# PalamaraLab/FastSMC

Hardware: NVIDIA B200
Metric: hmm_pair_sites_per_s (higher is better)
Workload: dtype f32

## Files before the change

fastsmc_b200/csrc/capi.cu:

```cuda
#include <algorithm>
#include <atomic>
#include <cub/device/device_radix_sort.cuh>
#include <chrono>
#include <cstdarg>
#include <cstdint>
#include <cstdio>
#include <cstdlib>
#include <cstring>
#include <map>
#include <tuple>
#include <numeric>
#include <string>
#include <thread>
#include <vector>

#include "decode_kernels.cuh"
#include "decode_fast.cuh"
#include "decode_sparse.cuh"
#include "seed_kernels.cuh"
#include "seed_order.h"
#include "host/SeedMapOrder.hpp"
#include "segment_sort.h"
#include "split_select.h"

// ... 71 lines not shown
    if (e == cudaSuccess) {
      n = want;
    }
    return e;
  }
};

}

struct fsmc_plan;

struct SeedKey {
  int32_t gap;
  float minLengthCm;
  uint64_t genPosSum, globalIdSum, flipSum;
  float skip;
  uint32_t window[4];
  int32_t lastJob, aboveDiag;
  uint32_t flags;
  int32_t maxSeeds, readAhead;
};

struct fsmc_ctx {
  int device = 0;
  cudaStream_t ownStream = nullptr;
  cudaStream_t stream = nullptr;
  cudaDeviceProp prop{};
  bool hasModel = false, hasHaps = false;
  uint64_t modelTag = 0;
  fsmc::DeviceModel model{};
  fsmc::DeviceModel kernelModel{};
  DevBuf<float> kernelSiteRows;
  DevBuf<float> laneAux;
  DevBuf<float> siteRows, prior, expTimes, colRatios;
  DevBuf<uint64_t> haps;
  long long numHaps = 0;
  DevBuf<float> scratch, accScratch;
  DevBuf<float> stageE1, stageE0, stageE2, stageD, stageB, stageU, stageR;
  DevBuf<int> stageRowIdx;
  DevBuf<float> sumScratch;
  DevBuf<float> ckptBeta;
  std::vector<float> hostPrior, hostExpTimes, hostColRatios;
  long long sites = 0;
  DevBuf<uint64_t> seedKeysT;
  DevBuf<uint32_t> seedOwner, seedSlotCount, seedSlotGroup, seedSlotOf, seedRankOf, seedMembers, seedGroupSize,
      seedGroupMemberBase, seedGlobalId;
  DevBuf<unsigned long long> seedGroupPairBase, seedCounters, seedWordCounters, seedChunkBase;
  DevBuf<float> seedGenPos;
  DevBuf<fsmc_match> seedOut;
  DevBuf<uint32_t> seedRank;
  DevBuf<unsigned char> seedLowComplexity;
  DevBuf<uint32_t> seedRep0, seedCur;
  DevBuf<unsigned char> seedDepth;
  DevBuf<uint64_t> seedRegKeyT, seedRegKeys;
  fsmc::CandidateOrderer orderer;
  const fsmc_match* orderedOut = nullptr;
  bool seedCacheValid = false;
  SeedKey seedCacheKey{};
  fsmc_seed_stats seedCacheStats{};
  cudaEvent_t ev[4] = {nullptr, nullptr, nullptr, nullptr};
  PinnedBuf<fsmc_segment> segStage;
  std::vector<uint32_t> pairOffset, pairFirst;
  fsmc::SegmentSorter segmentSorter;
  fsmc_plan* sparePlan = nullptr;
  std::map<std::tuple<const void*, int, size_t>, int> occupancy;
};
// ... 105 lines not shown
    }
    return {};
  }
  const bool acc = (flags & FSMC_SEG_AGE) && (flags & FSMC_CALL_SEGMENTS);
  const bool narrow = !(flags & (FSMC_SITE_MEAN | FSMC_SITE_MAP | FSMC_WIDE_KERNEL)) && (!acc || m.ageThreshold <= m.stateThreshold) &&
                      m.stateThreshold + 1 <= 4 * fsmc::kNarrowMaxQuads;
  const int rqWanted = narrow ? (m.stateThreshold + 1 + 3) / 4 : 0;
  const int pref = (flags & FSMC_ONE_WARP_KERNEL) ? 0 : splitPreference();
  const bool trySplit = pref == 1 || (pref == -1 && S == 159);
  if (trySplit && (S == 69 || S == 159) && m.stateThreshold <= 32) {
    fsmc::SplitChoice sc{};
    static const bool laneOff = [] { const char* e = std::getenv("FSMC_LANE"); return e && *e == '0'; }();
    if (S == 159 && m.laneAux && !laneOff) {
      sc = fsmc::laneKernel159(rqWanted);
    }
    if (!sc.fn) {
      sc = S == 69 ? fsmc::splitKernel69(rqWanted, acc) : fsmc::splitKernel159(rqWanted, acc);
    }
    if (!sc.fn && narrow) {
      sc = S == 69 ? fsmc::splitKernel69(0, acc) : fsmc::splitKernel159(0, acc);
    }
    if (sc.fn) {
      FastChoice fc{sc.fn, sc.Spad, sc.warps * 32, sc.acc, sc.recordQuads > 0, sc.recordQuads};
      fc.splitWarps = sc.warps;
      fc.splitSmem = sc.smemBytes;
      return fc;
    }
  }
  const bool sparse = preferSparse && S == 69 && acc && m.ageThreshold > m.stateThreshold &&
                      !(flags & (FSMC_SITE_MEAN | FSMC_SITE_MAP | FSMC_WIDE_KERNEL)) && m.stateThreshold + 1 <= 4 * fsmc::kNarrowMaxQuads;
  if (sparse) {
    const int rq = (m.stateThreshold + 1 + 3) / 4;
    FastKernelFn fn = rq == 1   ? fsmc::decodeNarrowKernel<69, 1, 4, kFastDepth, 128, 2, 1>
                      : rq == 2 ? fsmc::decodeNarrowKernel<69, 2, 4, kFastDepth, 128, 2, 1>
                      : rq == 3 ? fsmc::decodeNarrowKernel<69, 3, 2, kFastDepth, 128, 2, 1>
                                : fsmc::decodeNarrowKernel<69, 4, 2, kFastDepth, 128, 2, 1>;
    if (const char* e = std::getenv("FSMC_SPARSE_VARIANT")) {
      const int v = std::atoi(e);
      if (rq == 1 && v == 65) fn = fsmc::decodeNarrowKernel<69, 1, 4, kFastDepth, 128, 2, 65>;
    }
    FastChoice fc{fn, 72, 128, false, true, rq};
    fc.sparse = true;
    return fc;
  }
  if (S == 69 && narrow) {
    const int rq = (m.stateThreshold + 1 + 3) / 4;
    FastKernelFn fn = rq == 1   ? fsmc::decodeNarrowKernel<69, 1, 4, kFastDepth, 128, 2>
                      : rq == 2 ? fsmc::decodeNarrowKernel<69, 2, 4, kFastDepth, 128, 2>
                      : rq == 3 ? fsmc::decodeNarrowKernel<69, 3, 2, kFastDepth, 128, 2>
                                : fsmc::decodeNarrowKernel<69, 4, 2, kFastDepth, 128, 2>;
    if (const char* e = std::getenv("FSMC_SPARSE_VARIANT")) {
      if (rq == 1 && std::atoi(e) == 65) fn = fsmc::decodeNarrowKernel<69, 1, 4, kFastDepth, 128, 2, 64>;
    }
    return FastChoice{fn, 72, 128, false, true, rq};
  }
  if (S == 69) {
    return acc ? FastChoice{fsmc::decodeFastKernel<69, kFastDepth, kFastRescale, true, 128, 2>, 72, 128, true}
               : FastChoice{fsmc::decodeFastKernel<69, kFastDepth, kFastRescale, false, 128, 2>, 72, 128, false};
  }
  return {};
}
bool sparsePreferred(const double meanScanSites)
{
  if (const char* e = std::getenv("FSMC_SPARSE")) {
    return std::atoi(e) != 0;
  }
  return meanScanSites >= 2000.0;
}

size_t fastSmemBytes(const FastChoice& fc, const int S)
{
  if (fc.splitWarps > 0) {
    return fc.splitSmem;
  }
  const size_t warps = fc.threads / 32;
  if (fc.narrow) {
    const size_t group = fc.recordQuads <= 2 ? 4 : 2;
    const size_t slot = group * static_cast<size_t>(fsmc::kRowArrays) * fc.Spad * 4 + (group + 1) * static_cast<size_t>(fc.recordQuads) * 32 * 16;
    return warps * kFastDepth * slot + warps * kFastDepth * sizeof(uint64_t);
  }
  return warps * (kFastDepth * (static_cast<size_t>(fc.Spad) * 32 * 4 + static_cast<size_t>(fsmc::kRowArrays) * fc.Spad * 4) +
                  0 * static_cast<size_t>(S)) +
         warps * 2 * kFastDepth * sizeof(uint64_t);
}

size_t sumPosteriorCount(const DeviceModel& m, const unsigned flags)
{
  return static_cast<size_t>((flags & FSMC_SUM_BY_GENOTYPE) ? 3 : 1) * static_cast<size_t>(m.S) * static_cast<size_t>(m.L);
}

size_t smemPerWarp(const DeviceModel& m, const int mode, const unsigned flags)
{
  const bool age = (flags & FSMC_SEG_AGE) && (flags & FSMC_CALL_SEGMENTS);
  const size_t rows = (age ? m.ageThreshold : 0) + (mode >= 1 ? m.S : 0) + (mode == 2 ? m.S : 0);
  return rows * 32 * sizeof(float);
}

}

extern "C" {

const char* fsmc_last_error(void)
{
  return gLastError.c_str();
}

int fsmc_version(void)
{
  return 100;
}

// ... 147 lines not shown
  const int threads = 256;
  const int blocks = std::max(1, ctx->prop.multiProcessorCount * 8);
  fsmc::buildSiteRowsKernel<<<blocks, threads, 0, st>>>(S, Spad, L, e1.p, e0.p, e2.p, D.p, B.p, U.p, R.p, rowIdx.p,
                                                         ctx->siteRows.p);
  FSMC_CUDA(cudaGetLastError());
  FSMC_CUDA(cudaStreamSynchronize(st));

  DeviceModel& m = ctx->model;
  m.S = S;
  m.Spad = Spad;
  m.L = L;
  m.siteRows = ctx->siteRows.p;
  m.prior = ctx->prior.p;
  m.expTimes = ctx->expTimes.p;
  m.colRatios = ctx->colRatios.p;
  setThresholds(m);
  m.haps = ctx->haps.p;
  m.wordsPerHap = ctx->hasHaps ? (ctx->sites + 63) / 64 : 0;
  ctx->kernelModel = m;
  const int Sk = S <= 69 ? 69 : (S <= 159 ? 159 : 0);
  if (Sk != 0 && Sk != S) {
    const int SpadK = (Sk + 3) / 4 * 4;
    FSMC_CUDA(ctx->kernelSiteRows.ensure(static_cast<size_t>(L) * fsmc::kRowArrays * SpadK));
    fsmc::buildSiteRowsKernel<<<blocks, threads, 0, st>>>(S, SpadK, L, e1.p, e0.p, e2.p, D.p, B.p, U.p, R.p, rowIdx.p,
                                                           ctx->kernelSiteRows.p);
    FSMC_CUDA(cudaGetLastError());
    FSMC_CUDA(cudaStreamSynchronize(st));
    ctx->kernelModel.S = Sk;
    ctx->kernelModel.Spad = SpadK;
    ctx->kernelModel.siteRows = ctx->kernelSiteRows.p;
  }
  ctx->model.laneAux = nullptr;
  ctx->kernelModel.laneAux = nullptr;
  if (ctx->kernelModel.S == 159) {
    FSMC_CUDA(ctx->laneAux.ensure(static_cast<size_t>(L) * fsmc::laneAuxFloats159()));
    fsmc::buildLaneAux159(L, ctx->kernelModel.siteRows, ctx->laneAux.p, blocks, st);
    FSMC_CUDA(cudaGetLastError());
    FSMC_CUDA(cudaStreamSynchronize(st));
    ctx->kernelModel.laneAux = ctx->laneAux.p;
  }
  ctx->hasModel = true;
  ctx->modelTag = mdl->modelTag;
  return FSMC_OK;
}

int fsmc_set_haplotypes(fsmc_ctx* ctx, const uint64_t* bits, const int64_t numHaps, const int64_t sites)
{
  if (!ctx || !bits || numHaps < 1 || sites < 1) {
    return fail(FSMC_E_INVALID, "fsmc_set_haplotypes: bad argument");
  }
  FSMC_CUDA(cudaSetDevice(ctx->device));
  const long long words = (sites + 63) / 64;
  const size_t n = static_cast<size_t>(numHaps) * words;
  FSMC_CUDA(ctx->haps.ensure(n));
  FSMC_CUDA(cudaMemcpyAsync(ctx->haps.p, bits, n * sizeof(uint64_t), cudaMemcpyHostToDevice, ctx->stream));
  FSMC_CUDA(cudaStreamSynchronize(ctx->stream));
  ctx->model.haps = ctx->haps.p;
  ctx->model.wordsPerHap = words;
  ctx->kernelModel.haps = ctx->haps.p;
  ctx->kernelModel.wordsPerHap = words;
  ctx->numHaps = numHaps;
  ctx->sites = sites;
  ctx->hasHaps = true;
  ctx->seedCacheValid = false;
  return FSMC_OK;
}
// ... 990 lines not shown
```

fastsmc_b200/csrc/decode_fast.cuh:

```cuda
#pragma once

#include "decode_kernels.cuh"

namespace fsmc
{

constexpr int kMaxParamStates = 160;

struct FastModel {
  DeviceModel base;
  float colRatios[kMaxParamStates];
  float expTimes[kMaxParamStates];
  float prior[kMaxParamStates];
};

__device__ __forceinline__ uint32_t smemPtr(const void* p)
{
  return static_cast<uint32_t>(__cvta_generic_to_shared(p));
}
__device__ __forceinline__ void mbarInit(uint64_t* bar, const uint32_t count)
{
  asm volatile("mbarrier.init.shared::cta.b64 [%0], %1;" ::"r"(smemPtr(bar)), "r"(count) : "memory");
}
__device__ __forceinline__ void mbarExpectTx(uint64_t* bar, const uint32_t bytes)
// ... 248 lines not shown
          const float2 t = __fmul2_rn(pk(f4(u4, 2 * jp), f4(u4, 2 * jp + 1)), xx);
          const float au0 = au;
          const float au1 = fmaf(colRatios[k], au0, t.x);
          au = fmaf(colRatios[k1], au1, t.y);
          const float2 tt = __ffma2_rn(pk(f4(d4, 2 * jp), f4(d4, 2 * jp + 1)), xx, pk(au0, au1));
          const float2 w = __fmul2_rn(pk(f4(e4, 2 * jp), f4(e4, 2 * jp + 1)),
                                      __ffma2_rn(pk(f4(b4, 2 * jp), f4(b4, 2 * jp + 1)), pk(y[k], y[k1]), tt));
          y[k] = w.x;
          y[k1] = w.y;
        } else if (k < S) {
          y[k] = f4(e4, 2 * jp) * fmaf(f4(d4, 2 * jp), x[k], au);
        }
      }
    }
    {
      const int ql = QM - 1 - i;
      const float4 e4 = E[ql], b4 = Br[ql];
#pragma unroll
      for (int jp = 1; jp >= 0; --jp) {
        const int k = 4 * ql + 2 * jp, k1 = k + 1;
        const float s1 = run;
        const float s0 = s1 + x[k1];
        run = s0 + x[k];
        const float2 w = __fmul2_rn(pk(f4(e4, 2 * jp), f4(e4, 2 * jp + 1)),
                                    __ffma2_rn(pk(f4(b4, 2 * jp), f4(b4, 2 * jp + 1)), pk(s0, s1), pk(y[k], y[k1])));
        y[k] = w.x;
        y[k1] = w.y;
      }
    }
  }
  return run;
}

static __device__ __noinline__ int emitSparseItems(SparseItem* items, float* itemAlpha, unsigned long long* itemCount,
                                            const long long capacity, const bool pred, const uint32_t pair, const int block,
                                            const int first, const int last, int chain, const float4* alphaStart,
                                            const int lane, const int SQ)
{
  const unsigned mask = __ballot_sync(kFull, pred);
  if (!mask) {
    return chain;
  }
  unsigned long long base = 0;
  if (lane == 0) {
    base = atomicAdd(itemCount, static_cast<unsigned long long>(__popc(mask)));
  }
  base = __shfl_sync(kFull, base, 0);
  if (pred) {
    const long long slot = static_cast<long long>(base) + __popc(mask & ((1u << lane) - 1u));
    if (slot < capacity) {
      items[slot] = SparseItem{pair, block, first, last, chain};
      float4* dst = reinterpret_cast<float4*>(itemAlpha + static_cast<size_t>(slot) * SQ * 4);
      for (int q = 0; q < SQ; ++q) {
        dst[q] = alphaStart[q * 32 + lane];
      }
    }
    chain = static_cast<int>(slot);
  }
  return chain;
}

constexpr int kNarrowMaxQuads = 4;
constexpr int kNarrowGroup = 4;

template <int S_T, int RQ, int G> struct NarrowSlot {
  static constexpr int SQ = (S_T + 3) / 4, Spad = SQ * 4;
  static constexpr uint32_t kCoefBytes = kRowArrays * Spad * 4;
  static constexpr uint32_t kRecBytes = RQ * 32 * 16;
  static constexpr uint32_t kBytes = G * kCoefBytes + (G + 1) * kRecBytes;
};

template <int S_T, int RQ, int G, int DEPTH, int THREADS, int MIN_BLOCKS, int SPARSE_V = 0>
__global__ void __launch_bounds__(THREADS, MIN_BLOCKS) decodeNarrowKernel(const FastModel fm, const DecodeArgs args)
{
  constexpr bool SPARSE = (SPARSE_V & 1) != 0;
  constexpr bool kSkipFwd = (SPARSE_V & 2) != 0, kSkipBwd = (SPARSE_V & 4) != 0;
  constexpr int kGroupUnroll = (SPARSE_V & 64) ? G / 2 : 1;
  constexpr bool kSkipAlpha = (SPARSE_V & 8) != 0, kSkipBoundaryItems = (SPARSE_V & 16) != 0, kSkipRunItems = (SPARSE_V & 32) != 0;
  constexpr int S = S_T;
  constexpr int SQ = (S + 3) / 4;
  constexpr int Spad = SQ * 4;
  constexpr int NR = 4 * RQ - 1;
  using Slot = NarrowSlot<S_T, RQ, G>;
  constexpr uint32_t kRecBytes = Slot::kRecBytes;
  constexpr uint32_t kCoefBytes = Slot::kCoefBytes;
  constexpr size_t kRecFloats = static_cast<size_t>(RQ) * 32 * 4;
  constexpr size_t kRowFloats = static_cast<size_t>(kRowArrays) * Spad;
  constexpr int kWarps = THREADS / 32;
  constexpr size_t kWarpBytes = static_cast<size_t>(DEPTH) * Slot::kBytes;
  static_assert(S >= 4 * kNarrowMaxQuads && RQ >= 1 && RQ <= kNarrowMaxQuads, "record quads index the state vector");
  static_assert(G % 2 == 0, "the two state vectors swap roles every step");

  extern __shared__ __align__(128) unsigned char smemRaw[];
  const DeviceModel m = fm.base;
  const int lane = threadIdx.x & 31;
  const int warp = threadIdx.x >> 5;
  unsigned char* mine = smemRaw + static_cast<size_t>(warp) * kWarpBytes;
  uint64_t* bars = reinterpret_cast<uint64_t*>(smemRaw + static_cast<size_t>(kWarps) * kWarpBytes) + warp * DEPTH;
  auto coefArea = [&](const int slot) { return reinterpret_cast<float*>(mine + static_cast<size_t>(slot) * Slot::kBytes); };
  auto recArea = [&](const int slot) {
    return reinterpret_cast<float4*>(mine + static_cast<size_t>(slot) * Slot::kBytes + static_cast<size_t>(G) * kCoefBytes);
  };
  if (lane == 0) {
    for (int i = 0; i < DEPTH; ++i) {
      mbarInit(&bars[i], 1);
    }
    asm volatile("fence.mbarrier_init.release.cluster;" ::: "memory");
  }
  __syncwarp();
  uint32_t parity = 0;

  const unsigned flags = args.flags;
  const bool wantSeg = flags & FSMC_CALL_SEGMENTS;
  const bool wantAge = !SPARSE && (flags & FSMC_SEG_AGE) && wantSeg;
  const int sT = m.stateThreshold;
  const long long warpGlobal = static_cast<long long>(blockIdx.x) * kWarps + warp;
  float* slab = args.scratch + warpGlobal * args.scratchPerWarp;
  constexpr size_t kVecFloats = static_cast<size_t>(SQ) * 32 * 4;
  const int ckShift = SPARSE ? args.ckptShift : 0;
  const int ckMask = (1 << ckShift) - 1;
// ... 34 lines not shown
    };

    float a[S], c[S];
    float acc[NR];
#pragma unroll
    for (int k = 0; k < NR; ++k) {
      acc[k] = 0.f;
    }

    auto stageRecord = [&](const float (&v)[S], float4* out, const float divisor) {
#pragma unroll
      for (int q = 0; q < RQ; ++q) {
        float w[4];
#pragma unroll
        for (int i = 0; i < 4; ++i) {
          const int k = 4 * q + i;
          w[i] = k == NR ? divisor : (k < sT ? v[k] : 0.f);
        }
        out[q * 32 + lane] = make_float4(w[0], w[1], w[2], w[3]);
      }
    };

    {
      const int steps = len - 1;
      const int first = SPARSE ? min(steps, (len % G) ? (len % G) : G) : G;
      const int nGroups = steps <= 0 ? 0 : 1 + (max(steps - first, 0) + G - 1) / G;
      auto groupBegin = [&](const int g) { return g == 0 ? 0 : first + (g - 1) * G; };
      auto prefetch = [&](const int g) {
        if (lane == 0) {
          const int j0 = groupBegin(g), j1 = min(steps, j0 + (g == 0 ? first : G));
          const int slot = g % DEPTH;
          const uint32_t bytes = static_cast<uint32_t>(j1 - j0) * kCoefBytes;
          mbarExpectTx(&bars[slot], bytes);
          bulkLoad(coefArea(slot), rowBase + static_cast<size_t>(len - j1) * kRowFloats, bytes, &bars[slot]);
        }
      };
      for (int g = 0; g < DEPTH && g < nGroups; ++g) {
        prefetch(g);
      }
#pragma unroll
      for (int k = 0; k < S; ++k) {
        a[k] = 1.f;
      }
      if constexpr (SPARSE) {
        storeCheckpoint(a, len - 1);
      }
      if (nGroups == 0) {
        stageRecord(a, recArea(0), 1.0f);
        fenceProxyAsync();
        __syncwarp();
        if (lane == 0) {
          bulkStore(slab, recArea(0), kRecBytes);
          bulkCommit();
        }
      }
      for (int g = 0; g < nGroups; ++g) {
        const int slot = g % DEPTH;
        const int j0 = groupBegin(g);
        const int n = min(g == 0 ? first : G, steps - j0);
        const float* coef = coefArea(slot);
        float4* stage = recArea(slot);
        if constexpr (SPARSE && !kSkipBwd) {
          if (g > 0 && ((len - 1 - j0) & ckMask) == ckMask) {
            storeCheckpoint(a, len - 1 - j0);
          }
        }
        if (lane == 0) {
          bulkWaitRead<DEPTH - 1>();
        }
        mbarWait(&bars[slot], (parity >> slot) & 1u);
        parity ^= 1u << slot;
        __syncwarp();
        if (g == 0) {
          stageRecord(a, stage + static_cast<size_t>(n) * RQ * 32, 1.0f);
        }
        auto step = [&](const int i, float (&x)[S], float (&y)[S], const bool rescale) {
          const int p = len - 2 - (j0 + i);
          const int cls = bits.cls(from + p + 1);
          backwardStep<S>(x, y, coef + static_cast<size_t>(n - 1 - i) * kRowFloats, cls);
          float divisor = 1.0f;
          if (rescale) {
            divisor = sumStates<S>(y);
            scaleStates<S>(y, 1.0f / divisor);
          }
          stageRecord(y, stage + static_cast<size_t>(n - 1 - i) * RQ * 32, divisor);
        };
#pragma unroll(kGroupUnroll)
        for (int i = 0; i < G; i += 2) {
          if (i < n) {
            step(i, a, c, false);
          }
          if (i + 1 < n) {
            step(i + 1, c, a, i + 1 == G - 1);
          }
        }
        fenceProxyAsync();
        __syncwarp();
        if (lane == 0) {
          const int j1 = j0 + n;
          bulkStore(slab + static_cast<size_t>(len - 1 - j1) * kRecFloats, stage,
                    static_cast<uint32_t>(n + (g == 0 ? 1 : 0)) * kRecBytes);
          bulkCommit();
        }
        if (g + DEPTH < nGroups) {
          prefetch(g + DEPTH);
        }
        if (SPARSE && g == 0 && (n & 1)) {
#pragma unroll
          for (int k = 0; k < S; ++k) {
            a[k] = c[k];
          }
        }
      }
      const int rest = SPARSE ? max(steps - first, 0) : steps;
      if (rest & 1) {
      } else {
#pragma unroll
        for (int k = 0; k < S; ++k) {
          c[k] = a[k];
        }
      }
      if (lane == 0) {
        bulkWaitAll<0>();
      }
      __syncwarp();
    }

    {
      const int nGroups = (len + G - 1) / G;
      auto prefetch = [&](const int g) {
        if (lane == 0) {
          const int p0 = g * G;
          const uint32_t n = static_cast<uint32_t>(min(G, len - p0));
          const int slot = g % DEPTH;
          mbarExpectTx(&bars[slot], n * (kCoefBytes + kRecBytes));
          bulkLoad(coefArea(slot), rowBase + static_cast<size_t>(p0) * kRowFloats, n * kCoefBytes, &bars[slot]);
          bulkLoad(recArea(slot), slab + static_cast<size_t>(p0) * kRecFloats, n * kRecBytes, &bars[slot]);
        }
      };
      for (int g = 0; g < DEPTH && g < nGroups; ++g) {
        prefetch(g);
      }
      CallerState cs;
      float Z = 1.f, bPrev = 1.f;
      bool runOpen = false;
      int pieceStart = 0, chain = -1;
      auto emitItems = [&](const bool pred, const int block, const int first, const int last) {
        chain = emitSparseItems(args.items, args.itemAlpha, args.itemCount, args.itemCapacity, pred, pair, block, first, last, chain,
                                alphaStart, lane, SQ);
      };

      auto consume = [&](const int p, const float (&v)[S], float4* rec) {
        const int site = from + p;
        float q[4 * RQ];
#pragma unroll
        for (int qq = 0; qq < RQ; ++qq) {
          const float4 r4 = rec[qq * 32 + lane];
#pragma unroll
          for (int i = 0; i < 4; ++i) {
            q[4 * qq + i] = f4(r4, i);
          }
        }
        bPrev = q[NR];
        float ibdRaw = 0.f;
#pragma unroll
        for (int k = 0; k < NR; ++k) {
          q[k] *= v[k];
          ibdRaw += q[k];
        }
        const float r = 1.0f / Z;
        const float ibd = ibdRaw * r;
        if ((flags & FSMC_SITE_IBD) && laneActive) {
          args.siteIbd[static_cast<size_t>(pair) * args.siteStride + p] = ibd;
        }
        const bool inScan = wantSeg && site >= scanFrom && site < scanTo;
        if (inScan) {
          int now = ibd >= m.thr[0] ? 0 : (ibd >= m.thr[1] ? 1 : (ibd >= m.thr[2] ? 2 : (ibd >= m.thr[3] ? 3 : -1)));
          if (!laneActive) {
            now = -1;
          }
          const bool changed = now != cs.level;
          const bool ending = changed && cs.level >= 0;
          const bool closing = now >= 0 && site == scanTo - 1;
          const float rr = now >= 0 ? r : 0.f;
          const float keep = changed ? 0.f : 1.f;
          if constexpr (SPARSE && !kSkipFwd) {
            if (__any_sync(kFull, ending || closing)) {
              if constexpr (!kSkipRunItems) {
                emitItems(ending && runOpen && pieceStart <= site - 1, (p - 1) >> ckShift, pieceStart, site - 1);
              }
              if (ending) {
                emitSegment<false>(m, args, pair, cs.start, site - 1, cs.prob, cs.level, nullptr, false, chain);
                chain = -1;
                runOpen = false;
              }
              if (now >= 0 && changed) {
                runOpen = true;
                pieceStart = site;
              }
              if constexpr (!kSkipRunItems) {
                emitItems(closing, p >> ckShift, pieceStart, site);
              }
              if (closing) {
                emitSegment<false>(m, args, pair, changed ? site : cs.start, site, changed ? ibd : cs.prob + ibd, now, nullptr,
                                   false, chain);
                chain = -1;
                runOpen = false;
              }
            } else if (now >= 0 && changed) {
              runOpen = true;
              pieceStart = site;
            }
          } else if (__any_sync(kFull, ending || closing)) {
            float* park = reinterpret_cast<float*>(rec) + lane;
            __syncwarp();
            if (wantAge) {
#pragma unroll
              for (int k = 0; k < NR; ++k) {
                park[k * 32] = acc[k];
              }
              __syncwarp();
            }
            if (ending) {
              emitSegment<false>(m, args, pair, cs.start, site - 1, cs.prob, cs.level, park, wantAge);
            }
            __syncwarp();
            if (wantAge) {
#pragma unroll
              for (int k = 0; k < NR; ++k) {
                acc[k] = fmaf(q[k], rr, keep * acc[k]);
                park[k * 32] = acc[k];
              }
              __syncwarp();
            }
            if (closing) {
              emitSegment<false>(m, args, pair, changed ? site : cs.start, site, changed ? ibd : cs.prob + ibd, now, park, wantAge);
            }
            __syncwarp();
          } else if (wantAge) {
#pragma unroll
            for (int k = 0; k < NR; ++k) {
              acc[k] = fmaf(q[k], rr, keep * acc[k]);
            }
          }
          cs.prob = (now >= 0 && !closing) ? (changed ? ibd : cs.prob + ibd) : 0.f;
          cs.start = (now >= 0 && changed) ? site : cs.start;
          cs.level = now;
        }
      };

      for (int g = 0; g < nGroups; ++g) {
        const int slot = g % DEPTH;
        const int p0 = g * G;
        const int n = min(G, len - p0);
        const float* coef = coefArea(slot);
        float4* recs = recArea(slot);
        mbarWait(&bars[slot], (parity >> slot) & 1u);
        parity ^= 1u << slot;
        if constexpr (SPARSE && !kSkipFwd) {
          if (g > 0 && (p0 & ckMask) == 0) {
            if constexpr (!kSkipBoundaryItems) {
              if (__any_sync(kFull, runOpen)) {
                emitItems(runOpen, (p0 - 1) >> ckShift, pieceStart, from + p0 - 1);
              }
            }
            pieceStart = from + p0;
            if constexpr (!kSkipAlpha) {
              storeVector(c, alphaStart);
            }
          }
        }
        auto step = [&](const int i, float (&x)[S], float (&y)[S], const bool rescale) {
          const int p = p0 + i;
          const int cls = bits.cls(from + p);
          const float total = forwardStep<S>(fm.colRatios, x, y, coef + static_cast<size_t>(i) * kRowFloats, cls);
          float sc = 1.0f;
          if (rescale) {
            sc = 1.0f / total;
            scaleStates<S>(y, sc);
          }
          Z *= bPrev * sc;
          consume(p, y, recs + static_cast<size_t>(i) * RQ * 32);
        };
#pragma unroll(kGroupUnroll)
        for (int i = 0; i < G; i += 2) {
          if (i == 0 && g == 0) {
            const int cls = bits.cls(from);
            const float4* E = reinterpret_cast<const float4*>(coef + cls * Spad);
            float z0 = 0.f, z1 = 0.f, z2 = 0.f, z3 = 0.f;
#pragma unroll
            for (int q = 0; q < SQ; ++q) {
              const float4 e4 = E[q];
#pragma unroll
              for (int j = 0; j < 4; ++j) {
                const int k = 4 * q + j;
                if (k < S) {
                  a[k] = fm.prior[k] * f4(e4, j);
                }
              }
              z0 = fmaf(a[4 * q], c[4 * q], z0);
              if (4 * q + 1 < S) z1 = fmaf(a[4 * q + 1], c[4 * q + 1], z1);
              if (4 * q + 2 < S) z2 = fmaf(a[4 * q + 2], c[4 * q + 2], z2);
              if (4 * q + 3 < S) z3 = fmaf(a[4 * q + 3], c[4 * q + 3], z3);
            }
            Z = (z0 + z1) + (z2 + z3);
            consume(0, a, recs);
          } else if (i < n) {
            step(i, c, a, false);
          }
          if (i + 1 < n) {
            step(i + 1, a, c, i + 1 == G - 1);
          }
        }
        __syncwarp();
        if (g + DEPTH < nGroups) {
          prefetch(g + DEPTH);
        }
      }
    }
    __syncwarp();
  }
}

template <int S_T, int DEPTH, int RESCALE, bool ACC, int THREADS, int MIN_BLOCKS, bool SUM = false>
__global__ void __launch_bounds__(THREADS, MIN_BLOCKS) decodeFastKernel(const FastModel fm, const DecodeArgs args)
{
  constexpr int S = S_T;
  constexpr int SQ = (S + 3) / 4;
  constexpr int Spad = SQ * 4;
  constexpr uint32_t kBetaBytes = SQ * 32 * 16;
  constexpr uint32_t kCoefBytes = kRowArrays * Spad * 4;
  constexpr size_t kBetaFloats = static_cast<size_t>(SQ) * 32 * 4;
  constexpr int kWarps = THREADS / 32;
  constexpr size_t kWarpBytes = static_cast<size_t>(DEPTH) * (kBetaBytes + kCoefBytes);

  extern __shared__ __align__(128) unsigned char smemRaw[];
  const DeviceModel m = fm.base;
  const int lane = threadIdx.x & 31;
  const int warp = threadIdx.x >> 5;
  unsigned char* mine = smemRaw + static_cast<size_t>(warp) * kWarpBytes;
  uint64_t* bars = reinterpret_cast<uint64_t*>(smemRaw + static_cast<size_t>(kWarps) * kWarpBytes) +
                   warp * 2 * DEPTH;
  auto betaSlot = [&](const int i) { return reinterpret_cast<float4*>(mine + static_cast<size_t>(i) * kBetaBytes); };
  auto coefSlot = [&](const int i) {
    return reinterpret_cast<const float*>(mine + static_cast<size_t>(DEPTH) * kBetaBytes + static_cast<size_t>(i) * kCoefBytes);
  };
  if (lane == 0) {
    for (int i = 0; i < 2 * DEPTH; ++i) {
      mbarInit(&bars[i], 1);
// ... 365 lines not shown
```

fastsmc_b200/csrc/decode_kernels.cuh:

```cuda
#pragma once

#include <cstdint>
#include <cuda_runtime.h>

#include "../../include/fastsmc_b200.h"

namespace fsmc
{

constexpr int kRowArrays = 8;
constexpr unsigned kFull = 0xffffffffu;

struct DeviceModel {
  int S;
  int Spad;
  int L;
  const float* siteRows;
  const float* laneAux;
  const float* prior;
  const float* expTimes;
  const float* colRatios;
  int stateThreshold;
  int ageThreshold;
  float thr[4];
  const uint64_t* haps;
  long long wordsPerHap;
};

struct SparseItem {
  uint32_t pair;
  int32_t block;
  int32_t first, last;
  int32_t prev;
};

struct DecodeArgs {
  const uint32_t* hapA;
  const uint32_t* hapB;
  const int* tilePairs;
  const int* tileFrom;
  const int* tileTo;
  const int* tileScanFrom;
  const int* tileScanTo;
  const int* order;
  long long numTiles;
  unsigned flags;
  fsmc_segment* segments;
  unsigned long long* segmentCount;
  long long segmentCapacity;
  float* siteMean;
// ... 512 lines not shown
                                    const int* __restrict__ distRow, float* __restrict__ rows)
{
  const long long total = static_cast<long long>(L) * Spad;
  for (long long i = blockIdx.x * static_cast<long long>(blockDim.x) + threadIdx.x; i < total;
       i += static_cast<long long>(gridDim.x) * blockDim.x) {
    const int site = static_cast<int>(i / Spad);
    const int k = static_cast<int>(i % Spad);
    float* out = rows + static_cast<size_t>(site) * kRowArrays * Spad + k;
    float v[kRowArrays] = {0.f, 0.f, 0.f, 0.f, 0.f, 0.f, 0.f, 0.f};
    if (k < S) {
      const size_t e = static_cast<size_t>(site) * S + k;
      const float hm = __fadd_rn(e1[e], e0m1[e]);
      v[0] = hm;
      v[1] = e1[e];
      v[2] = __fadd_rn(hm, e2m0[e]);
      if (site > 0) {
        const size_t t = static_cast<size_t>(distRow[site]) * S + k;
        v[3] = D[t];
        v[4] = B[t];
        v[5] = U[t];
        v[6] = RR[t];
        if (k > 0) {
          v[7] = U[t - 1];
        }
      }
    }
#pragma unroll
    for (int j = 0; j < kRowArrays; ++j) {
      out[static_cast<size_t>(j) * Spad] = v[j];
    }
  }
}

}
```

Before: 17.07 billion.

## Defer narrow-kernel segment emission to a per-group replay outside the hot loop

Instead of emitting segments and sparse items inline inside each per-site consume step (with warp votes and syncs), the kernel records per-site event bits and stashes the needed state into the record/spare smem slots, then replays all events once per group in a noinline helper. This is meant to drop divergent branches and warp syncs from the forward-step inner loop and shrink its register and code footprint. It also changes the default kernel path, because the consume rewrite applies to all variants, and it adds a kNoEvents (bit 128) benchmarking variant selectable via environment variable. The risk is extra shared-memory writes, and correctness depends on reusing the coef area as park space.

```diff
diff --git a/fastsmc_b200/csrc/capi.cu b/fastsmc_b200/csrc/capi.cu
--- a/fastsmc_b200/csrc/capi.cu
+++ b/fastsmc_b200/csrc/capi.cu
@@ -304,6 +304,7 @@
     if (const char* e = std::getenv("FSMC_SPARSE_VARIANT")) {
       const int v = std::atoi(e);
       if (rq == 1 && v == 65) fn = fsmc::decodeNarrowKernel<69, 1, 4, kFastDepth, 128, 2, 65>;
+      if (rq == 1 && v == 129) fn = fsmc::decodeNarrowKernel<69, 1, 4, kFastDepth, 128, 2, 129>;
     }
     FastChoice fc{fn, 72, 128, false, true, rq};
     fc.sparse = true;
@@ -316,7 +317,9 @@
                       : rq == 3 ? fsmc::decodeNarrowKernel<69, 3, 2, kFastDepth, 128, 2>
                                 : fsmc::decodeNarrowKernel<69, 4, 2, kFastDepth, 128, 2>;
     if (const char* e = std::getenv("FSMC_SPARSE_VARIANT")) {
-      if (rq == 1 && std::atoi(e) == 65) fn = fsmc::decodeNarrowKernel<69, 1, 4, kFastDepth, 128, 2, 64>;
+      const int v = std::atoi(e);
+      if (rq == 1 && v == 65) fn = fsmc::decodeNarrowKernel<69, 1, 4, kFastDepth, 128, 2, 64>;
+      if (rq == 1 && v == 129) fn = fsmc::decodeNarrowKernel<69, 1, 4, kFastDepth, 128, 2, 128>;
     }
     return FastChoice{fn, 72, 128, false, true, rq};
   }
diff --git a/fastsmc_b200/csrc/decode_fast.cuh b/fastsmc_b200/csrc/decode_fast.cuh
--- a/fastsmc_b200/csrc/decode_fast.cuh
+++ b/fastsmc_b200/csrc/decode_fast.cuh
@@ -332,6 +332,63 @@
   return chain;
 }
 
+template <bool SPARSE, bool RUN_ITEMS, int RQ, int G>
+static __device__ __noinline__ int replayNarrowEvents(const DeviceModel& m, const DecodeArgs& args, const uint32_t pair,
+                                                      const int lane, const unsigned events, const float4* recs,
+                                                      float* park, const float* closePark, const bool wantAge,
+                                                      const int from, const int p0, const int closeSite,
+                                                      const CallerState cs, const int pieceStart, int chain,
+                                                      const float4* alphaStart, const int ckShift, const int SQ)
+{
+  constexpr int NR = 4 * RQ - 1;
+  const unsigned all = __reduce_or_sync(kFull, events);
+  const float* spare = reinterpret_cast<const float*>(recs + G * RQ * 32 + lane);
+  for (int i = 0; i < G; ++i) {
+    if (!((all >> i) & 1u)) {
+      continue;
+    }
+    const bool ending = (events >> i) & 1u;
+    const float* e = reinterpret_cast<const float*>(recs + i * RQ * 32 + lane);
+    auto word = [&](const int k) { return e[(k / 4) * 128 + k % 4]; };
+    const int packed = __float_as_int(word(NR));
+    const int site = from + p0 + i;
+    if constexpr (SPARSE) {
+      if constexpr (RUN_ITEMS) {
+        const int first = __float_as_int(word(0));
+        chain = emitSparseItems(args.items, args.itemAlpha, args.itemCount, args.itemCapacity, ending && first <= site - 1,
+                                pair, (p0 + i - 1) >> ckShift, first, site - 1, chain, alphaStart, lane, SQ);
+      }
+      if (ending) {
+        emitSegment<false>(m, args, pair, packed >> 2, site - 1, spare[i], packed & 3, nullptr, false, chain);
+        chain = -1;
+      }
+    } else if (ending) {
+      if (wantAge) {
+        for (int k = 0; k < NR; ++k) {
+          park[k * 32 + lane] = word(k);
+        }
+      }
+      emitSegment<false>(m, args, pair, packed >> 2, site - 1, spare[i], packed & 3, park + lane, wantAge);
+    }
+  }
+  if ((all >> G) & 1u) {
+    const bool closing = (events >> G) & 1u;
+    if constexpr (SPARSE) {
+      if constexpr (RUN_ITEMS) {
+        chain = emitSparseItems(args.items, args.itemAlpha, args.itemCount, args.itemCapacity, closing, pair,
+                                (closeSite - from) >> ckShift, pieceStart, closeSite, chain, alphaStart, lane, SQ);
+      }
+      if (closing) {
+        emitSegment<false>(m, args, pair, cs.start, closeSite, cs.prob, cs.level, nullptr, false, chain);
+        chain = -1;
+      }
+    } else if (closing) {
+      emitSegment<false>(m, args, pair, cs.start, closeSite, cs.prob, cs.level, closePark + lane, wantAge);
+    }
+  }
+  return chain;
+}
+
 constexpr int kNarrowMaxQuads = 4;
 constexpr int kNarrowGroup = 4;
 
@@ -349,6 +406,9 @@
   constexpr bool kSkipFwd = (SPARSE_V & 2) != 0, kSkipBwd = (SPARSE_V & 4) != 0;
   constexpr int kGroupUnroll = (SPARSE_V & 64) ? G / 2 : 1;
   constexpr bool kSkipAlpha = (SPARSE_V & 8) != 0, kSkipBoundaryItems = (SPARSE_V & 16) != 0, kSkipRunItems = (SPARSE_V & 32) != 0;
+  constexpr bool kNoEvents = (SPARSE_V & 128) != 0;
+  constexpr bool kSparseFwd = SPARSE && !kSkipFwd;
+  static_assert(G <= 4, "one word of the spare record per position of the group");
   constexpr int S = S_T;
   constexpr int SQ = (S + 3) / 4;
   constexpr int Spad = SQ * 4;
@@ -575,8 +635,10 @@
         chain = emitSparseItems(args.items, args.itemAlpha, args.itemCount, args.itemCapacity, pred, pair, block, first, last, chain,
                                 alphaStart, lane, SQ);
       };
-
-      auto consume = [&](const int p, const float (&v)[S], float4* rec) {
+      unsigned events = 0;
+      [[maybe_unused]] unsigned sink = 0;
+
+      auto consume = [&](const int i, const int p, const float (&v)[S], float4* rec) {
         const int site = from + p;
         float q[4 * RQ];
 #pragma unroll
@@ -608,69 +670,39 @@
           const bool changed = now != cs.level;
           const bool ending = changed && cs.level >= 0;
           const bool closing = now >= 0 && site == scanTo - 1;
+          const bool starting = now >= 0 && changed;
           const float rr = now >= 0 ? r : 0.f;
           const float keep = changed ? 0.f : 1.f;
-          if constexpr (SPARSE && !kSkipFwd) {
-            if (__any_sync(kFull, ending || closing)) {
-              if constexpr (!kSkipRunItems) {
-                emitItems(ending && runOpen && pieceStart <= site - 1, (p - 1) >> ckShift, pieceStart, site - 1);
+          if constexpr (!kNoEvents) {
+            float w[4 * RQ];
+#pragma unroll
+            for (int k = 0; k < NR; ++k) {
+              w[k] = kSparseFwd ? (k == 0 ? __int_as_float(runOpen ? pieceStart : INT_MAX) : 0.f) : acc[k];
+            }
+            w[NR] = __int_as_float((cs.start << 2) | cs.level);
+#pragma unroll
+            for (int qq = 0; qq < RQ; ++qq) {
+              if ((!kSparseFwd || qq == 0 || qq == RQ - 1) && ending) {
+                rec[qq * 32 + lane] = make_float4(w[4 * qq], w[4 * qq + 1], w[4 * qq + 2], w[4 * qq + 3]);
               }
-              if (ending) {
-                emitSegment<false>(m, args, pair, cs.start, site - 1, cs.prob, cs.level, nullptr, false, chain);
-                chain = -1;
-                runOpen = false;
-              }
-              if (now >= 0 && changed) {
-                runOpen = true;
-                pieceStart = site;
-              }
-              if constexpr (!kSkipRunItems) {
-                emitItems(closing, p >> ckShift, pieceStart, site);
-              }
-              if (closing) {
-                emitSegment<false>(m, args, pair, changed ? site : cs.start, site, changed ? ibd : cs.prob + ibd, now, nullptr,
-                                   false, chain);
-                chain = -1;
-                runOpen = false;
-              }
-            } else if (now >= 0 && changed) {
-              runOpen = true;
-              pieceStart = site;
-            }
-          } else if (__any_sync(kFull, ending || closing)) {
-            float* park = reinterpret_cast<float*>(rec) + lane;
-            __syncwarp();
-            if (wantAge) {
-#pragma unroll
-              for (int k = 0; k < NR; ++k) {
-                park[k * 32] = acc[k];
-              }
-              __syncwarp();
             }
             if (ending) {
-              emitSegment<false>(m, args, pair, cs.start, site - 1, cs.prob, cs.level, park, wantAge);
-            }
-            __syncwarp();
-            if (wantAge) {
-#pragma unroll
-              for (int k = 0; k < NR; ++k) {
-                acc[k] = fmaf(q[k], rr, keep * acc[k]);
-                park[k * 32] = acc[k];
-              }
-              __syncwarp();
-            }
-            if (closing) {
-              emitSegment<false>(m, args, pair, changed ? site : cs.start, site, changed ? ibd : cs.prob + ibd, now, park, wantAge);
-            }
-            __syncwarp();
-          } else if (wantAge) {
+              reinterpret_cast<float*>(rec + (G - i) * RQ * 32 + lane)[i] = cs.prob;
+            }
+          }
+          events |= (ending ? 1u << i : 0u) | (closing ? 1u << G : 0u);
+          if (wantAge) {
 #pragma unroll
             for (int k = 0; k < NR; ++k) {
               acc[k] = fmaf(q[k], rr, keep * acc[k]);
             }
           }
-          cs.prob = (now >= 0 && !closing) ? (changed ? ibd : cs.prob + ibd) : 0.f;
-          cs.start = (now >= 0 && changed) ? site : cs.start;
+          if constexpr (kSparseFwd) {
+            runOpen = changed ? now >= 0 : runOpen;
+            pieceStart = starting ? site : pieceStart;
+          }
+          cs.prob = now >= 0 ? (changed ? ibd : cs.prob + ibd) : 0.f;
+          cs.start = starting ? site : cs.start;
           cs.level = now;
         }
       };
@@ -706,7 +738,7 @@
             scaleStates<S>(y, sc);
           }
           Z *= bPrev * sc;
-          consume(p, y, recs + static_cast<size_t>(i) * RQ * 32);
+          consume(i, p, y, recs + static_cast<size_t>(i) * RQ * 32);
         };
 #pragma unroll(kGroupUnroll)
         for (int i = 0; i < G; i += 2) {
@@ -730,7 +762,7 @@
               if (4 * q + 3 < S) z3 = fmaf(a[4 * q + 3], c[4 * q + 3], z3);
             }
             Z = (z0 + z1) + (z2 + z3);
-            consume(0, a, recs);
+            consume(0, 0, a, recs);
           } else if (i < n) {
             step(i, c, a, false);
           }
@@ -739,8 +771,39 @@
           }
         }
         __syncwarp();
+        if constexpr (kNoEvents) {
+          sink |= events;
+        } else if (__any_sync(kFull, events != 0)) {
+          float* park = const_cast<float*>(coef);
+          float* closePark = park + 16 * 32;
+          if (!kSparseFwd && wantAge && ((events >> G) & 1u)) {
+#pragma unroll
+            for (int k = 0; k < NR; ++k) {
+              closePark[k * 32 + lane] = acc[k];
+            }
+          }
+          chain = replayNarrowEvents<kSparseFwd, !kSkipRunItems, RQ, G>(m, args, pair, lane, events, recs, park, closePark,
+                                                                        wantAge, from, p0, scanTo - 1, cs, pieceStart, chain,
+                                                                        alphaStart, ckShift, SQ);
+          if ((events >> G) & 1u) {
+            runOpen = false;
+          }
+          fenceProxyAsync();
+          __syncwarp();
+        }
+        events = 0;
         if (g + DEPTH < nGroups) {
           prefetch(g + DEPTH);
+        }
+      }
+      if constexpr (kNoEvents) {
+#pragma unroll
+        for (int k = 0; k < NR; ++k) {
+          sink ^= __float_as_uint(acc[k]);
+        }
+        sink ^= __float_as_uint(cs.prob) ^ static_cast<unsigned>(cs.start) ^ static_cast<unsigned>(pieceStart) ^ (runOpen ? 1u : 0u);
+        if (sink == 0xffffffffu && __float_as_uint(Z) == 0xffffffffu) {
+          *args.segmentCount = sink;
         }
       }
     }
```

Result: faster. 17.41 billion (median of 6 runs) (+2.0%).

## Precompute emission-folded backward coefficient rows and use folded backward step in narrow kernel

Applied to the files above, without the earlier changes.

Adds a per-site table built once at model setup that holds emission probabilities already multiplied into the U, D and B transition coefficients for each of the three genotype classes, plus the R row. The narrow kernel's backward pass streams these rows and runs a new folded backward step that processes the upper and lower state halves together with packed f32x2 math, removing per-step emission multiplies. The cost is larger coefficient slots (10 arrays instead of 8) in shared memory and bulk loads, so the rq==2 variant's group size drops from 4 to 2 to fit. The forward pass keeps loading the original rows.

```diff
diff --git a/fastsmc_b200/csrc/capi.cu b/fastsmc_b200/csrc/capi.cu
--- a/fastsmc_b200/csrc/capi.cu
+++ b/fastsmc_b200/csrc/capi.cu
@@ -127,6 +127,7 @@
   fsmc::DeviceModel kernelModel{};
   DevBuf<float> kernelSiteRows;
   DevBuf<float> laneAux;
+  DevBuf<float> bwdRows;
   DevBuf<float> siteRows, prior, expTimes, colRatios;
   DevBuf<uint64_t> haps;
   long long numHaps = 0;
@@ -298,7 +299,7 @@
   if (sparse) {
     const int rq = (m.stateThreshold + 1 + 3) / 4;
     FastKernelFn fn = rq == 1   ? fsmc::decodeNarrowKernel<69, 1, 4, kFastDepth, 128, 2, 1>
-                      : rq == 2 ? fsmc::decodeNarrowKernel<69, 2, 4, kFastDepth, 128, 2, 1>
+                      : rq == 2 ? fsmc::decodeNarrowKernel<69, 2, 2, kFastDepth, 128, 2, 1>
                       : rq == 3 ? fsmc::decodeNarrowKernel<69, 3, 2, kFastDepth, 128, 2, 1>
                                 : fsmc::decodeNarrowKernel<69, 4, 2, kFastDepth, 128, 2, 1>;
     if (const char* e = std::getenv("FSMC_SPARSE_VARIANT")) {
@@ -312,7 +313,7 @@
   if (S == 69 && narrow) {
     const int rq = (m.stateThreshold + 1 + 3) / 4;
     FastKernelFn fn = rq == 1   ? fsmc::decodeNarrowKernel<69, 1, 4, kFastDepth, 128, 2>
-                      : rq == 2 ? fsmc::decodeNarrowKernel<69, 2, 4, kFastDepth, 128, 2>
+                      : rq == 2 ? fsmc::decodeNarrowKernel<69, 2, 2, kFastDepth, 128, 2>
                       : rq == 3 ? fsmc::decodeNarrowKernel<69, 3, 2, kFastDepth, 128, 2>
                                 : fsmc::decodeNarrowKernel<69, 4, 2, kFastDepth, 128, 2>;
     if (const char* e = std::getenv("FSMC_SPARSE_VARIANT")) {
@@ -341,8 +342,8 @@
   }
   const size_t warps = fc.threads / 32;
   if (fc.narrow) {
-    const size_t group = fc.recordQuads <= 2 ? 4 : 2;
-    const size_t slot = group * static_cast<size_t>(fsmc::kRowArrays) * fc.Spad * 4 + (group + 1) * static_cast<size_t>(fc.recordQuads) * 32 * 16;
+    const size_t group = fc.recordQuads == 1 ? 4 : 2;
+    const size_t slot = group * static_cast<size_t>(fsmc::kBwdArrays) * fc.Spad * 4 + (group + 1) * static_cast<size_t>(fc.recordQuads) * 32 * 16;
     return warps * kFastDepth * slot + warps * kFastDepth * sizeof(uint64_t);
   }
   return warps * (kFastDepth * (static_cast<size_t>(fc.Spad) * 32 * 4 + static_cast<size_t>(fsmc::kRowArrays) * fc.Spad * 4) +
@@ -556,6 +557,15 @@
   }
   ctx->model.laneAux = nullptr;
   ctx->kernelModel.laneAux = nullptr;
+  ctx->model.bwdRows = nullptr;
+  ctx->kernelModel.bwdRows = nullptr;
+  if (ctx->kernelModel.S == 69) {
+    FSMC_CUDA(ctx->bwdRows.ensure(static_cast<size_t>(L) * fsmc::kBwdArrays * ctx->kernelModel.Spad));
+    fsmc::buildBackwardRowsKernel<<<blocks, threads, 0, st>>>(ctx->kernelModel.Spad, L, ctx->kernelModel.siteRows, ctx->bwdRows.p);
+    FSMC_CUDA(cudaGetLastError());
+    FSMC_CUDA(cudaStreamSynchronize(st));
+    ctx->kernelModel.bwdRows = ctx->bwdRows.p;
+  }
   if (ctx->kernelModel.S == 159) {
     FSMC_CUDA(ctx->laneAux.ensure(static_cast<size_t>(L) * fsmc::laneAuxFloats159()));
     fsmc::buildLaneAux159(L, ctx->kernelModel.siteRows, ctx->laneAux.p, blocks, st);
diff --git a/fastsmc_b200/csrc/decode_fast.cuh b/fastsmc_b200/csrc/decode_fast.cuh
--- a/fastsmc_b200/csrc/decode_fast.cuh
+++ b/fastsmc_b200/csrc/decode_fast.cuh
@@ -304,6 +304,102 @@
   return run;
 }
 
+template <int S>
+__device__ __forceinline__ void backwardStepFolded(const float (&x)[S], float (&y)[S], const float* row, const int cls)
+{
+  constexpr int SQ = (S + 3) / 4, Spad = SQ * 4, QM = (SQ + 1) / 2;
+  static_assert(4 * QM < S - 1, "the lower half lies below the last state");
+  const float4* UsE = reinterpret_cast<const float4*>(row + cls * Spad);
+  const float4* DE = reinterpret_cast<const float4*>(row + (3 + cls) * Spad);
+  const float4* BE = reinterpret_cast<const float4*>(row + (6 + cls) * Spad);
+  const float4* Rr = reinterpret_cast<const float4*>(row + 9 * Spad);
+  float bu = 0.f, bl = 0.f;
+  float above = 0.f;
+#pragma unroll
+  for (int i = 0; i < QM; ++i) {
+    const int qu = SQ - 1 - i;
+    if (qu >= QM) {
+      const float4 u4 = UsE[qu], r4 = Rr[qu];
+#pragma unroll
+      for (int jp = 1; jp >= 0; --jp) {
+        const int k = 4 * qu + 2 * jp, k1 = k + 1;
+        if (k1 < S) {
+          const float2 t = __fmul2_rn(pk(f4(u4, 2 * jp), f4(u4, 2 * jp + 1)), pk(x[k], x[k1]));
+          if (k1 == S - 1) {
+            y[k1] = 0.f;
+          } else {
+            bu = fmaf(f4(r4, 2 * jp + 1), bu, above);
+            y[k1] = bu;
+          }
+          bu = fmaf(f4(r4, 2 * jp), bu, t.y);
+          y[k] = bu;
+          above = t.x;
+        } else if (k < S) {
+          above = f4(u4, 2 * jp) * x[k];
+          if (k == S - 1) {
+            y[k] = 0.f;
+          } else {
+            bu = fmaf(f4(r4, 2 * jp), bu, above);
+            y[k] = bu;
+          }
+        }
+      }
+    }
+    {
+      const int ql = i;
+      const float4 d4 = DE[ql], b4 = BE[ql];
+#pragma unroll
+      for (int jp = 0; jp < 2; ++jp) {
+        const int k = 4 * ql + 2 * jp, k1 = k + 1;
+        const float bl0 = bl;
+        const float bl1 = fmaf(f4(b4, 2 * jp), x[k], bl0);
+        bl = fmaf(f4(b4, 2 * jp + 1), x[k1], bl1);
+        const float2 w = __ffma2_rn(pk(f4(d4, 2 * jp), f4(d4, 2 * jp + 1)), pk(x[k], x[k1]), pk(bl0, bl1));
+        y[k] = w.x;
+        y[k1] = w.y;
+      }
+    }
+  }
+#pragma unroll
+  for (int i = 0; i < QM; ++i) {
+    {
+      const int ql = QM - 1 - i;
+      const float4 u4 = UsE[ql], r4 = Rr[ql];
+#pragma unroll
+      for (int jp = 1; jp >= 0; --jp) {
+        const int k = 4 * ql + 2 * jp, k1 = k + 1;
+        const float2 t = __fmul2_rn(pk(f4(u4, 2 * jp), f4(u4, 2 * jp + 1)), pk(x[k], x[k1]));
+        const float b1 = fmaf(f4(r4, 2 * jp + 1), bu, above);
+        const float b0 = fmaf(f4(r4, 2 * jp), b1, t.y);
+        bu = b0;
+        above = t.x;
+        const float2 w = __fadd2_rn(pk(y[k], y[k1]), pk(b0, b1));
+        y[k] = w.x;
+        y[k1] = w.y;
+      }
+    }
+    const int qu = QM + i;
+    if (qu < SQ) {
+      const float4 d4 = DE[qu], b4 = BE[qu];
+#pragma unroll
+      for (int jp = 0; jp < 2; ++jp) {
+        const int k = 4 * qu + 2 * jp, k1 = k + 1;
+        if (k1 < S) {
+          const float bl0 = bl;
+          const float bl1 = fmaf(f4(b4, 2 * jp), x[k], bl0);
+          bl = fmaf(f4(b4, 2 * jp + 1), x[k1], bl1);
+          const float2 w = __fadd2_rn(__ffma2_rn(pk(f4(d4, 2 * jp), f4(d4, 2 * jp + 1)), pk(x[k], x[k1]), pk(bl0, bl1)),
+                                      pk(y[k], y[k1]));
+          y[k] = w.x;
+          y[k1] = w.y;
+        } else if (k < S) {
+          y[k] = fmaf(f4(d4, 2 * jp), x[k], bl) + y[k];
+        }
+      }
+    }
+  }
+}
+
 static __device__ __noinline__ int emitSparseItems(SparseItem* items, float* itemAlpha, unsigned long long* itemCount,
                                             const long long capacity, const bool pred, const uint32_t pair, const int block,
                                             const int first, const int last, int chain, const float4* alphaStart,
@@ -337,7 +433,7 @@
 
 template <int S_T, int RQ, int G> struct NarrowSlot {
   static constexpr int SQ = (S_T + 3) / 4, Spad = SQ * 4;
-  static constexpr uint32_t kCoefBytes = kRowArrays * Spad * 4;
+  static constexpr uint32_t kCoefBytes = kBwdArrays * Spad * 4;
   static constexpr uint32_t kRecBytes = RQ * 32 * 16;
   static constexpr uint32_t kBytes = G * kCoefBytes + (G + 1) * kRecBytes;
 };
@@ -358,6 +454,8 @@
   constexpr uint32_t kCoefBytes = Slot::kCoefBytes;
   constexpr size_t kRecFloats = static_cast<size_t>(RQ) * 32 * 4;
   constexpr size_t kRowFloats = static_cast<size_t>(kRowArrays) * Spad;
+  constexpr uint32_t kRowBytes = static_cast<uint32_t>(kRowFloats) * 4;
+  constexpr size_t kBwdFloats = static_cast<size_t>(kBwdArrays) * Spad;
   constexpr int kWarps = THREADS / 32;
   constexpr size_t kWarpBytes = static_cast<size_t>(DEPTH) * Slot::kBytes;
   static_assert(S >= 4 * kNarrowMaxQuads && RQ >= 1 && RQ <= kNarrowMaxQuads, "record quads index the state vector");
@@ -458,7 +556,7 @@
           const int slot = g % DEPTH;
           const uint32_t bytes = static_cast<uint32_t>(j1 - j0) * kCoefBytes;
           mbarExpectTx(&bars[slot], bytes);
-          bulkLoad(coefArea(slot), rowBase + static_cast<size_t>(len - j1) * kRowFloats, bytes, &bars[slot]);
+          bulkLoad(coefArea(slot), m.bwdRows + static_cast<size_t>(from + len - j1) * kBwdFloats, bytes, &bars[slot]);
         }
       };
       for (int g = 0; g < DEPTH && g < nGroups; ++g) {
@@ -503,7 +601,7 @@
         auto step = [&](const int i, float (&x)[S], float (&y)[S], const bool rescale) {
           const int p = len - 2 - (j0 + i);
           const int cls = bits.cls(from + p + 1);
-          backwardStep<S>(x, y, coef + static_cast<size_t>(n - 1 - i) * kRowFloats, cls);
+          backwardStepFolded<S>(x, y, coef + static_cast<size_t>(n - 1 - i) * kBwdFloats, cls);
           float divisor = 1.0f;
           if (rescale) {
             divisor = sumStates<S>(y);
@@ -559,8 +657,8 @@
           const int p0 = g * G;
           const uint32_t n = static_cast<uint32_t>(min(G, len - p0));
           const int slot = g % DEPTH;
-          mbarExpectTx(&bars[slot], n * (kCoefBytes + kRecBytes));
-          bulkLoad(coefArea(slot), rowBase + static_cast<size_t>(p0) * kRowFloats, n * kCoefBytes, &bars[slot]);
+          mbarExpectTx(&bars[slot], n * (kRowBytes + kRecBytes));
+          bulkLoad(coefArea(slot), rowBase + static_cast<size_t>(p0) * kRowFloats, n * kRowBytes, &bars[slot]);
           bulkLoad(recArea(slot), slab + static_cast<size_t>(p0) * kRecFloats, n * kRecBytes, &bars[slot]);
         }
       };
diff --git a/fastsmc_b200/csrc/decode_kernels.cuh b/fastsmc_b200/csrc/decode_kernels.cuh
--- a/fastsmc_b200/csrc/decode_kernels.cuh
+++ b/fastsmc_b200/csrc/decode_kernels.cuh
@@ -9,6 +9,7 @@
 {
 
 constexpr int kRowArrays = 8;
+constexpr int kBwdArrays = 10;
 constexpr unsigned kFull = 0xffffffffu;
 
 struct DeviceModel {
@@ -16,6 +17,7 @@
   int Spad;
   int L;
   const float* siteRows;
+  const float* bwdRows;
   const float* laneAux;
   const float* prior;
   const float* expTimes;
@@ -594,4 +596,26 @@
   }
 }
 
-}
+static __global__ void buildBackwardRowsKernel(const int Spad, const int L, const float* __restrict__ rows,
+                                               float* __restrict__ bwd)
+{
+  const long long total = static_cast<long long>(L) * Spad;
+  for (long long i = blockIdx.x * static_cast<long long>(blockDim.x) + threadIdx.x; i < total;
+       i += static_cast<long long>(gridDim.x) * blockDim.x) {
+    const int site = static_cast<int>(i / Spad);
+    const int k = static_cast<int>(i % Spad);
+    const float* r = rows + static_cast<size_t>(site) * kRowArrays * Spad + k;
+    const float D = r[3 * Spad], B = r[4 * Spad], Us = r[7 * Spad];
+    float* b = bwd + static_cast<size_t>(site) * kBwdArrays * Spad + k;
+#pragma unroll
+    for (int c = 0; c < 3; ++c) {
+      const float e = r[c * Spad];
+      b[c * Spad] = __fmul_rn(Us, e);
+      b[(3 + c) * Spad] = __fmul_rn(D, e);
+      b[(6 + c) * Spad] = __fmul_rn(B, e);
+    }
+    b[9 * Spad] = r[6 * Spad];
+  }
+}
+
+}
```

Result: faster. 17.10 billion before, 17.72 billion after (median of 6 runs) (+3.6%).
